# zhu-xlab/PFST

Hardware: AMD Instinct MI355X
Metric: PFST train-step images/s on 1024² IRRG tiles (higher is better)
Workload: dtype f32 (f16x3 split MFMA: two scaled fp16 pieces per operand, three products, fp32 accumulate); 1 GPU; pfst_pots_irrg2vaih_irrg_deeplabv3plus_r50-d8; global_batch=8, per_gpu_batch=8, tile=1024x1024x3, num_classes=6, parallelism=dp1, weights=seeded random init, conv_math=f16x3

## Files before the change

pfst_amd/csrc/conv_f16x3.hip:

```cpp
#include "conv_epilogue.h"
#include "amax.h"
#include "det.h"
#include "weight_jobs.h"
#include <math.h>
#include <stdlib.h>
#include <type_traits>
#include <utility>
#include "../../include/pfst_hip.h"

typedef _Float16 f16x8 __attribute__((ext_vector_type(8)));
typedef float f32x4 __attribute__((ext_vector_type(4)));

namespace {

constexpr int BN = 128;
constexpr int NP = 2;

template <int... Is, class F>
__device__ __forceinline__ void static_for_seq(std::integer_sequence<int, Is...>, F&& f) {
  (f(std::integral_constant<int, Is>()), ...);
}
template <int N, class F>
__device__ __forceinline__ void static_for(F&& f) {
  static_for_seq(std::make_integer_sequence<int, N>(), static_cast<F&&>(f));
// ... 73 lines not shown
  else if constexpr (op == 4)
    asm volatile("v_fma_mixlo_f16 %0, %1, %2, -%3 op_sel:[0,0,0] op_sel_hi:[0,0,1]" : "=v"(st.l[q]) : "v"(v[2 * q]), "s"(s), "v"(st.h[q]));
  else if constexpr (op == 5)
    asm volatile("v_fma_mixhi_f16 %0, %1, %2, -%3 op_sel:[0,0,1] op_sel_hi:[0,0,1]" : "+v"(st.l[q]) : "v"(v[2 * q + 1]), "s"(s), "v"(st.h[q]));
}
#endif

template <int K>
__device__ __forceinline__ void unpack_op_f16(const float (&v)[8], SplitF16& st) {
  constexpr int q = K & 3;
  if constexpr (K < 4) asm volatile("v_perm_b32 %0, %1, %2, %3" : "=v"(st.h[q]) : "v"(v[2 * q + 1]), "v"(v[2 * q]), "s"(0x05040100u));
  else asm volatile("v_perm_b32 %0, %1, %2, %3" : "=v"(st.l[q]) : "v"(v[2 * q + 1]), "v"(v[2 * q]), "s"(0x07060302u));
}

__global__ void pack_weight_f16x2_kernel(const float* __restrict__ w, uint4* __restrict__ wf, uint4* __restrict__ wd, int Cout, int Cin, int T,
                                         i64 set_in, i64 set_out, const float* __restrict__ amax) {
  w += blockIdx.y * set_in;
  if (wf) wf += blockIdx.y * set_out;
  if (wd) wd += blockIdx.y * set_out;
  const float s = scale_of(amax_exponent(amax_read(amax + (i64)blockIdx.y * PFST_AMAX_SUB)));
  const i64 nf = (i64)(T * Cin / 16) * 2 * Cout, nd = (i64)(T * Cout / 16) * 2 * Cin;
  for (i64 i = (i64)blockIdx.x * blockDim.x + threadIdx.x; i < nf + nd; i += (i64)gridDim.x * blockDim.x) {
    const bool dg = i >= nf;
    const i64 e = dg ? i - nf : i;
    const int M = dg ? Cin : Cout, Cq = dg ? Cout : Cin;
    if ((dg ? wd : wf) == nullptr) continue;
    if (Cq % 16 != 0) continue;
    const int row = (int)(e % M);
    const i64 gh = e / M;
    const int h = (int)(gh & 1);
    const int g = (int)(gh >> 1);
    float v[8];
#pragma unroll
    for (int j = 0; j < 8; ++j) {
      const int k = g * 16 + h * 8 + j;
      const int t = k / Cq, c = k - t * Cq;
      const int co = dg ? c : row, ci = dg ? row : c;
      v[j] = w[((i64)co * Cin + ci) * T + t];
    }
    uint4 ph, pl;
    split8_f16(v, s, ph, pl);
    uint4* dst = dg ? wd : wf;
    const i64 base = (i64)g * 2 * NP * M;
    dst[base + (i64)(0 * 2 + h) * M + row] = ph;
    dst[base + (i64)(1 * 2 + h) * M + row] = pl;
  }
}

__global__ __launch_bounds__(256) void pack_weight_f16x2_batched_kernel(const pfst_weight_job_t* __restrict__ jobs, int njobs) {
  const pfst_weight_job_t J = jobs[weight_job_of_block(jobs, njobs, blockIdx.x)];
  const int lb = blockIdx.x - J.first_block;
  const int Cout = J.Cout, Cin = J.Cin, T = J.T;
  const i64 nf = J.dst_f ? (i64)(T * Cin / 16) * 2 * Cout : 0, nd = J.dst_d ? (i64)(T * Cout / 16) * 2 * Cin : 0;
  const int bps = (int)((nf + nd + 255) / 256);
  const int set = lb / bps;
  const i64 n = (i64)Cout * Cin * T;
  const float s = scale_of(amax_exponent(amax_read(J.amax_f + (i64)set * PFST_AMAX_SUB)));
  const i64 i = (i64)(lb - set * bps) * 256 + threadIdx.x;
  if (i >= nf + nd) return;
  const float* w = J.src + set * n;
  const bool dg = i >= nf;
  const i64 e = dg ? i - nf : i;
  const int M = dg ? Cin : Cout, Cq = dg ? Cout : Cin;
  const int row = (int)(e % M);
  const i64 gh = e / M;
  const int h = (int)(gh & 1);
  const int g = (int)(gh >> 1);
  float v[8];
#pragma unroll
  for (int j = 0; j < 8; ++j) {
    const int k = g * 16 + h * 8 + j;
    const int t = k / Cq, c = k - t * Cq;
    const int co = dg ? c : row, ci = dg ? row : c;
    v[j] = w[((i64)co * Cin + ci) * T + t];
  }
  uint4 ph, pl;
  split8_f16(v, s, ph, pl);
  uint4* dst = reinterpret_cast<uint4*>(dg ? J.dst_d : J.dst_f) + set * (4 * n / 16);
  const i64 base = (i64)g * 2 * NP * M;
  dst[base + (i64)(0 * 2 + h) * M + row] = ph;
  dst[base + (i64)(1 * 2 + h) * M + row] = pl;
}

struct PfstResGate {
  const float* g = nullptr;
  i64 g_bs = 0;
  const unsigned long long* mask = nullptr;
};

template <int SHAPE, int BNB = 0, bool BPACK = false, bool ONE = false, int BMT = 128, bool BNL = false>
__device__ __forceinline__ void conv_igemm_f16x3_body(
    const float* __restrict__ in, i64 in_bs, const uint4* __restrict__ wk4, const float* __restrict__ bias,
    float* __restrict__ out, i64 out_bs, int C, int Hi, int Wi, int M, int Ho, int Wo, int ks,
    int ca, int cb, int cc, int cdivv, int accumulate, float* __restrict__ stats, int stats_T,
    const float* __restrict__ w_amax, const float* __restrict__ in_amax, int Y, int Z, int chain, const PfstBnbArgs& bnb,
    const PfstResGate& gate, const float4* __restrict__ bnl = nullptr) {
  static_assert(!BNL || (BMT == 256 && ONE && !BPACK && BNB == 0), "normalise-on-load exists for the 256-row 1x1 forward tile");
  static_assert(SHAPE == 32, "one MFMA shape: v_mfma_f32_32x32x16_f16 (the 16x16x32 form of round 3 was removed in round 5)");
  static_assert(BMT == 128 || (BMT == 256 && SHAPE == 32 && ONE) || (BMT == 64 && SHAPE == 32 && BNB == 0 && !BPACK),
                "the 256-row tile exists for the pixel-to-pixel 32x32 loop, the 64-row tile for the plain 32x32 loop");
  constexpr int BM = BMT, WAVES_N = 2, NT = BM == 64 ? 256 : 2 * BM;
  constexpr int TMW = BM == 64 ? 1 : 2;
  constexpr int TPT = BM == 256 ? 1 : 2;
  constexpr int NA = 2 * (2 * NP * BM) / NT;
  constexpr int TILE_A = 2 * NP * BM, TILE_B = 2 * NP * BN;
  constexpr int PAIR_CHUNKS = 2 * TILE_A + 2 * TILE_B;
  constexpr int SMEM_CHUNKS = 2 * PAIR_CHUNKS;
  __shared__ uint4 smem[SMEM_CHUNKS];
  uint4* const As = smem;
  uint4* const Bs = smem + 2 * TILE_A;

  const int tid = threadIdx.x, lane = tid & 63, wid = __builtin_amdgcn_readfirstlane(tid >> 6);
  const int wm0 = (wid / WAVES_N) * (32 * TMW), wn0 = (wid % WAVES_N) * 64;
  const int P = Ho * Wo, HiWi = Hi * Wi;
  constexpr int BNL_ROWS = 2048 + 32;
  __shared__ uint4 bnl_s[BNL ? BNL_ROWS / 2 : 1];
  if constexpr (BNL) {
    for (int i = tid; i < BNL_ROWS; i += NT) {
      const float4 cf = i < C ? bnl[i] : make_float4(0.f, 0.f, 0.f, 0.f);
      reinterpret_cast<float2*>(bnl_s)[i] = make_float2(cf.z, cf.w);
    }
    __syncthreads();
  }
  const int gx = (P + BN - 1) / BN, gy = (M + BM - 1) / BM, X = gx * gy;
  const int total = X * Y * Z, G = gridDim.x;
  auto decode = [&](int lin, int& bx, int& by, int& y, int& n) {
    const int zy = lin / X, x = lin - zy * X;
    y = zy / Z;
    const int z = zy - y * Z;
    n = y * Z + z;
    pfst_tile_order(x, gx, gy, !ONE && ks == 3, bx, by);
  };
  const int spt = (C + 31) / 32;
  const int ntaps = ONE ? 1 : ks * ks;
  const int KP = spt * ntaps;
  const int KT16 = (C / 16) * ntaps;
  const bool CHAIN = ONE && SHAPE == 32 && (KP & 1) == 0 && (chain & 1) != 0;
  float* const stats_mm = (stats && (chain & 2)) ? stats + (i64)2 * M * stats_T : nullptr;
#ifdef PFST_NT_ALL_K
  const bool nt_out = (chain & 4) != 0;
#else
  const bool nt_out = KP <= 16 && (chain & 4) != 0;
#endif

  const int pix = tid & (BN - 1), kh = (tid >> 7) & 1;
  const int bt = BM == 256 ? tid >> 8 : 0;
  const int a_seg = tid / BM, a_row = tid - a_seg * BM;
  constexpr unsigned OOB = 0x80000000u;
  const int a_chunk = 2 * M * 16, a_tile = 2 * NP * M * 16, b_chan = HiWi * 4;
  const int chan_step = 32 * HiWi * 4;

  int ld_lin = blockIdx.x;
  __amdgpu_buffer_rsrc_t a_rsrc, b_rsrc;
  unsigned a_voff;
  int ld_oy, ld_ox;
  bool ld_pvalid;
  auto set_load_side = [&](int lin) {
    int bx, by, y, n;
    decode(lin, bx, by, y, n);
    const int p = bx * BN + pix, m0 = by * BM;
    ld_pvalid = p < P;
    if constexpr (ONE) {
      ld_oy = p;
      ld_ox = 0;
    } else {
      ld_oy = ld_pvalid ? p / Wo : 0;
      ld_ox = ld_pvalid ? p - ld_oy * Wo : 0;
    }
    a_voff = (m0 + a_row < M) ? 16u * ((unsigned)a_seg * (unsigned)M + (unsigned)(m0 + a_row)) : OOB;
    a_rsrc = __builtin_amdgcn_make_buffer_rsrc(const_cast<uint4*>(wk4) + (i64)y * KT16 * 2 * NP * M, 0, KT16 * 2 * NP * M * 16, 0x00020000);
    b_rsrc = __builtin_amdgcn_make_buffer_rsrc(const_cast<float*>(in) + (i64)n * in_bs, 0, C * HiWi * 4, 0x00020000);
  };
  auto tap_voff = [&](int tap) -> unsigned {
    if constexpr (ONE) return ld_pvalid ? 4u * ((unsigned)(bt * 16 + kh * 8) * (unsigned)HiWi + (unsigned)ld_oy) : OOB;
    const int ty = tap / ks, tx = tap - ty * ks;
    int sy, sx;
    const bool ok = ld_pvalid & src_coord(ld_oy, ty, ca, cb, cc, cdivv, Hi, sy) & src_coord(ld_ox, tx, ca, cb, cc, cdivv, Wi, sx);
    return ok ? 4u * ((unsigned)(kh * 8) * (unsigned)HiWi + (unsigned)(sy * Wi + sx)) : OOB;
  };

  uint4 areg[2][NA];
  float breg[2][TPT][8];
  pfst_f32x16 acc32[TMW][2];
#pragma unroll
  for (int i = 0; i < TMW; ++i)
#pragma unroll
    for (int j = 0; j < 2; ++j)
#pragma unroll
      for (int r = 0; r < 16; ++r) acc32[i][j][r] = 0.f;

  auto load_b = [&](auto vc, auto setc, unsigned voff, int soff) {
    constexpr int v = decltype(vc)::value, SET = decltype(setc)::value;
    breg[SET][v >> 3][v & 7] = __builtin_bit_cast(float, __builtin_amdgcn_raw_buffer_load_b32(b_rsrc, voff, soff + ((v >> 3) * 16 + (v & 7)) * b_chan, 0));
  };
  auto load_a = [&](auto vc, auto setc, int a_soff) {
    constexpr int v = decltype(vc)::value, SET = decltype(setc)::value;
    areg[SET][v] = __builtin_bit_cast(uint4, __builtin_amdgcn_raw_buffer_load_b128(a_rsrc, a_voff, a_soff + (v / (NA / 2)) * a_tile + (v % (NA / 2)) * a_chunk, 0));
// ... 83 lines not shown
    uint4 cfr[BNL ? 4 : 1];
    const int cf_at = BNL ? sidx1 * 16 + bt * 8 + kh * 4 : 0;
    auto filler = [&](auto sc) {
      constexpr int m = decltype(sc)::value;
      if constexpr (m < 8) {
        if constexpr (TPT == 2) {
          load_b(std::integral_constant<int, 2 * m>(), std::integral_constant<int, SETL>(), voff2, soff2);
          load_b(std::integral_constant<int, 2 * m + 1>(), std::integral_constant<int, SETL>(), voff2, soff2);
        } else {
          load_b(std::integral_constant<int, m>(), std::integral_constant<int, SETL>(), voff2, soff2);
        }
      }
      if constexpr (m >= 8 && m < 8 + NA) As[NXT + ((m - 8) / (NA / 2)) * TILE_A + tid + NT * ((m - 8) % (NA / 2))] = areg[SETN][m - 8];
      if constexpr (BNL && m >= 8 && m < 12) cfr[m - 8] = bnl_s[cf_at + (m - 8)];
      if constexpr (m >= 12) {
        constexpr int SPS = 2 * TPT;
        static_for<SPS>([&](auto kc) {
          constexpr int kk = (m - 12) * SPS + decltype(kc)::value;
          if constexpr (BPACK) {
            if constexpr (kk < 8) unpack_op_f16<kk>(breg[SETN][0], s0);
            else if constexpr (kk < 16 && TPT == 2) unpack_op_f16<kk - 8>(breg[SETN][TPT - 1], s1);
          } else {
            if constexpr (BNL && kk < 24 && kk % 6 < 2) {
              constexpr int e = 2 * (kk / 6) + kk % 6;
              const uint4 c2 = cfr[e >> 1];
              const float sc = __builtin_bit_cast(float, (e & 1) ? c2.z : c2.x), sh = __builtin_bit_cast(float, (e & 1) ? c2.w : c2.y);
              breg[SETN][0][e] = fmaxf(__fmaf_rn(breg[SETN][0][e], sc, sh), 0.f);
            }
            if constexpr (kk < 24) split_op_f16<kk>(breg[SETN][0], sb, s0);
            else split_op_f16<kk - 24>(breg[SETN][TPT - 1], sb, s1);
          }
        });
      }
      if constexpr (m >= 12 && m < 12 + NA) load_a(std::integral_constant<int, m - 12>(), std::integral_constant<int, SETL>(), a_soff2);
      if constexpr (m == 18 && TPT == 2) {
        Bs[NXT + (0 * 2 + kh) * BN + pix] = make_uint4(s0.h[0], s0.h[1], s0.h[2], s0.h[3]);
        Bs[NXT + (1 * 2 + kh) * BN + pix] = make_uint4(s0.l[0], s0.l[1], s0.l[2], s0.l[3]);
      }
      if constexpr (m == 23 && TPT == 2) {
        Bs[NXT + TILE_B + (0 * 2 + kh) * BN + pix] = make_uint4(s1.h[0], s1.h[1], s1.h[2], s1.h[3]);
        Bs[NXT + TILE_B + (1 * 2 + kh) * BN + pix] = make_uint4(s1.l[0], s1.l[1], s1.l[2], s1.l[3]);
      }
      if constexpr (m == 23 && TPT == 1) {
        Bs[NXT + bt * TILE_B + (0 * 2 + kh) * BN + pix] = make_uint4(s0.h[0], s0.h[1], s0.h[2], s0.h[3]);
        Bs[NXT + bt * TILE_B + (1 * 2 + kh) * BN + pix] = make_uint4(s0.l[0], s0.l[1], s0.l[2], s0.l[3]);
      }
    };
    static_for<12 * TMW>([&](auto mc) {
      constexpr int m = decltype(mc)::value;
      constexpr int prod = m / (4 * TMW), rem = m % (4 * TMW), t = rem / (2 * TMW), i = (rem >> 1) % TMW, j = rem & 1;
      constexpr int pa = prod == 0 ? 1 : 0, pb = prod == 1 ? 1 : 0;
      acc32[i][j] = __builtin_amdgcn_mfma_f32_32x32x16_f16(af[t][i][pa], bf[t][j][pb], acc32[i][j], 0, 0, 0);
      if constexpr (PRE + m < 4 * RG) read_frag(std::integral_constant<int, PRE + m>());
      if constexpr (TMW == 2) {
        filler(std::integral_constant<int, m>());
      } else {
        filler(std::integral_constant<int, 2 * m>());
        filler(std::integral_constant<int, 2 * m + 1>());
      }
      __builtin_amdgcn_sched_barrier(0);
    });
    advance();
    __syncthreads();
  };
  auto epilogue = [&](int lin) {
    int bx, by, y, n;
    decode(lin, bx, by, y, n);
    if (y != ea_y) {
      ea = amax_exponent(amax_read(w_amax + (i64)y * PFST_AMAX_SUB));
      ea_y = y;
    }
    const int p0 = bx * BN, m0 = by * BM;
    float* const outn = out + (i64)n * out_bs;
    const float* const gsrc = gate.g ? gate.g + (i64)n * gate.g_bs : nullptr;
    const unsigned long long* const gmask = gate.g ? gate.mask + (i64)n * M * (P >> 6) : nullptr;
    const float ua = unscale_of(ea), ub = unscale_of(eb);
    {
#pragma unroll
      for (int i = 0; i < TMW; ++i)
#pragma unroll
        for (int j = 0; j < 2; ++j)
#pragma unroll
          for (int r = 0; r < 16; ++r) acc32[i][j][r] = acc32[i][j][r] * ua * ub;
      if constexpr (BNB != 0) {
        static_assert(PAIR_CHUNKS * sizeof(uint4) >= (NT / 64) * PFST_ROWSUM_LDS_FLOATS * sizeof(float), "epilogue scratch must fit into one pair buffer");
        conv_epilogue<2, 2, WAVES_N, BN, BNB, true>(acc32, outn, bias, stats, stats_T, accumulate, M, P, m0, p0, wm0, wn0, bx, n, wid, lane, bnb,
                                                    reinterpret_cast<float*>(smem + PAIR_CHUNKS), gsrc, gmask, nullptr, nt_out);
        __syncthreads();
      } else {
#ifdef PFST_STATS_LDSRED
        if (stats && !stats_mm && BMT != 64) {
          conv_epilogue<TMW, 2, WAVES_N, BN, 0, true>(acc32, outn, bias, stats, stats_T, accumulate, M, P, m0, p0, wm0, wn0, bx, n, wid, lane, PfstBnbArgs(),
                                                      reinterpret_cast<float*>(smem + PAIR_CHUNKS), gsrc, gmask, nullptr, nt_out);
          __syncthreads();
        } else
#endif
        conv_epilogue<TMW, 2, WAVES_N, BN>(acc32, outn, bias, stats, stats_T, accumulate, M, P, m0, p0, wm0, wn0, bx, n, wid, lane, PfstBnbArgs(), nullptr,
                                           gsrc, gmask, stats_mm, nt_out);
      }
#pragma unroll
      for (int i = 0; i < TMW; ++i)
#pragma unroll
        for (int j = 0; j < 2; ++j)
#pragma unroll
          for (int r = 0; r < 16; ++r) acc32[i][j][r] = 0.f;
    }
  };

  for (int lin = blockIdx.x; lin < total; lin += G) {
    if (!CHAIN || lin == (int)blockIdx.x) prologue(lin);
    for (int k = 0; k < KP; k += 2) {
      step32(std::integral_constant<int, 1>(), k);
      if (k + 1 < KP) step32(std::integral_constant<int, 0>(), k + 1);
    }
    epilogue(lin);
  }
}

template <int SHAPE, bool BPACK = false, bool ONE = false, int BMT = 128>
__global__ __launch_bounds__(BMT == 64 ? 256 : 2 * BMT, BMT == 256 ? 1 : 2) void conv_igemm_f16x3_kernel(
    const float* __restrict__ in, i64 in_bs, const uint4* __restrict__ wk4, const float* __restrict__ bias,
    float* __restrict__ out, i64 out_bs, int C, int Hi, int Wi, int M, int Ho, int Wo, int ks,
    int ca, int cb, int cc, int cdivv, int accumulate, float* __restrict__ stats, int stats_T,
    const float* __restrict__ w_amax, const float* __restrict__ in_amax, int Y, int Z, int chain, PfstResGate gate) {
  conv_igemm_f16x3_body<SHAPE, 0, BPACK, ONE, BMT>(in, in_bs, wk4, bias, out, out_bs, C, Hi, Wi, M, Ho, Wo, ks, ca, cb, cc, cdivv, accumulate, stats, stats_T,
                               w_amax, in_amax, Y, Z, chain, PfstBnbArgs(), gate);
}
__global__ __launch_bounds__(512, 1) void conv_igemm_f16x3_bnl_kernel(
    const float* __restrict__ in, i64 in_bs, const uint4* __restrict__ wk4, const float* __restrict__ bias,
    float* __restrict__ out, i64 out_bs, int C, int Hi, int Wi, int M, int Ho, int Wo, int ks,
    int ca, int cb, int cc, int cdivv, int accumulate, float* __restrict__ stats, int stats_T,
    const float* __restrict__ w_amax, const float* __restrict__ in_amax, int Y, int Z, int chain, const float4* __restrict__ bnl) {
  conv_igemm_f16x3_body<32, 0, false, true, 256, true>(in, in_bs, wk4, bias, out, out_bs, C, Hi, Wi, M, Ho, Wo, ks, ca, cb, cc, cdivv, accumulate, stats,
                                                       stats_T, w_amax, in_amax, Y, Z, chain, PfstBnbArgs(), PfstResGate(), bnl);
}
template <int BNB, bool ONE = false, int BMT = 128>
__global__ __launch_bounds__(2 * BMT, BMT == 128 ? 2 : 1) void conv_igemm_f16x3_bnb_kernel(
    const float* __restrict__ in, i64 in_bs, const uint4* __restrict__ wk4, const float* __restrict__ bias,
    float* __restrict__ out, i64 out_bs, int C, int Hi, int Wi, int M, int Ho, int Wo, int ks,
    int ca, int cb, int cc, int cdivv, int accumulate, float* __restrict__ stats, int stats_T,
    const float* __restrict__ w_amax, const float* __restrict__ in_amax, int Y, int Z, int chain, PfstBnbArgs bnb, PfstResGate gate) {
  conv_igemm_f16x3_body<32, BNB, false, ONE, BMT>(in, in_bs, wk4, bias, out, out_bs, C, Hi, Wi, M, Ho, Wo, ks, ca, cb, cc, cdivv, accumulate, stats, stats_T,
                                 w_amax, in_amax, Y, Z, chain, bnb, gate);
}


typedef float f32x16 __attribute__((ext_vector_type(16)));

struct Split4 {
  unsigned h[2], l[2];
  float t0[2], t1[2];
};
#ifdef PFST_F16X3_SPLIT6
template <int K>
__device__ __forceinline__ void split4_op_f16(const float (&v)[4], float s, Split4& st) {
  constexpr int q = K / 6, op = K % 6;
  if constexpr (op == 0) asm volatile("v_mul_f32 %0, %1, %2" : "=v"(st.t0[q]) : "s"(s), "v"(v[2 * q]));
  else if constexpr (op == 1) asm volatile("v_mul_f32 %0, %1, %2" : "=v"(st.t1[q]) : "s"(s), "v"(v[2 * q + 1]));
  else if constexpr (op == 2) asm volatile("v_cvt_pk_f16_f32 %0, %1, %2" : "=v"(st.h[q]) : "v"(st.t0[q]), "v"(st.t1[q]));
  else if constexpr (op == 3)
    asm volatile("v_fma_mix_f32 %0, %1, %2, -%3 op_sel:[0,0,0] op_sel_hi:[0,0,1]" : "=v"(st.t0[q]) : "v"(v[2 * q]), "s"(s), "v"(st.h[q]));
  else if constexpr (op == 4)
    asm volatile("v_fma_mix_f32 %0, %1, %2, -%3 op_sel:[0,0,1] op_sel_hi:[0,0,1]" : "=v"(st.t1[q]) : "v"(v[2 * q + 1]), "s"(s), "v"(st.h[q]));
  else asm volatile("v_cvt_pk_f16_f32 %0, %1, %2" : "=v"(st.l[q]) : "v"(st.t0[q]), "v"(st.t1[q]));
}
#else
template <int K>
__device__ __forceinline__ void split4_op_f16(const float (&v)[4], float s, Split4& st) {
  constexpr int q = K / 6, op = K % 6;
  if constexpr (op == 2) asm volatile("v_fma_mixlo_f16 %0, %1, %2, 0 op_sel_hi:[0,0,0]" : "=v"(st.h[q]) : "v"(v[2 * q]), "s"(s));
  else if constexpr (op == 3) asm volatile("v_fma_mixhi_f16 %0, %1, %2, 0 op_sel_hi:[0,0,0]" : "+v"(st.h[q]) : "v"(v[2 * q + 1]), "s"(s));
  else if constexpr (op == 4)
    asm volatile("v_fma_mixlo_f16 %0, %1, %2, -%3 op_sel:[0,0,0] op_sel_hi:[0,0,1]" : "=v"(st.l[q]) : "v"(v[2 * q]), "s"(s), "v"(st.h[q]));
  else if constexpr (op == 5)
    asm volatile("v_fma_mixhi_f16 %0, %1, %2, -%3 op_sel:[0,0,1] op_sel_hi:[0,0,1]" : "+v"(st.l[q]) : "v"(v[2 * q + 1]), "s"(s), "v"(st.h[q]));
}
#endif
template <int K>
__device__ __forceinline__ void unpack4_op_f16(const float (&v)[4], Split4& st) {
  constexpr int q = K & 1;
  if constexpr (K < 2) asm volatile("v_perm_b32 %0, %1, %2, %3" : "=v"(st.h[q]) : "v"(v[2 * q + 1]), "v"(v[2 * q]), "s"(0x05040100u));
  else asm volatile("v_perm_b32 %0, %1, %2, %3" : "=v"(st.l[q]) : "v"(v[2 * q + 1]), "v"(v[2 * q]), "s"(0x07060302u));
}

template <bool PACK, int BMT = 128, bool BNL = false>
__global__ __launch_bounds__(2 * BMT, BMT == 128 ? 2 : 1) void conv_wgrad_f16x3_line_kernel(
    const float* __restrict__ x, i64 x_bs, const float* __restrict__ dy, i64 dy_bs, float* __restrict__ dw,
    int J, int M, int P, int chunks, int chunk_len, int N, i64 x_gs, i64 dy_gs, i64 dw_gs, int gx, int gy, int gz,
    const float* __restrict__ x_amax, const float* __restrict__ dy_amax, const float4* __restrict__ bnl) {
  static_assert(!BNL || !PACK, "a pre-split operand is already normalised");
  constexpr int BM = BMT, BJ = 128, WM = 64, WAVES_N = 2, WN = 64, TM = 2, TN = 2, NT = 2 * BM;
  constexpr int RPP = NT / 8;
  constexpr int PA = BM / RPP, PB = BJ / RPP;
  constexpr int ROWS_A = BM + 2, ROWS_B = BJ + 2;
  constexpr int TILE_A = 4 * ROWS_A + 4, TILE_B = 4 * ROWS_B + 4;
  __shared__ uint4 As[2][2 * TILE_A];
  __shared__ uint4 Bs[2][2 * TILE_B];

  const int tid = threadIdx.x, lane = tid & 63, wid = __builtin_amdgcn_readfirstlane(tid >> 6);
  const int wm0 = (wid / WAVES_N) * WM, wn0 = (wid % WAVES_N) * WN;
  int bx, by, bz;
  {
    const int lin = blockIdx.x, tiles = gx * gy, z8 = gz & ~7;
    if (lin < tiles * z8) {
      const int xcd = lin & 7, idx = lin >> 3;
      const int sl = idx / tiles, t = idx - sl * tiles;
      bz = sl * 8 + xcd;
      by = t / gx;
      bx = t - by * gx;
    } else {
      bz = lin / tiles;
      const int t = lin - bz * tiles;
      by = t / gx;
      bx = t - by * gx;
    }
  }
  const int j0 = bx * BJ, m0 = by * BM;
// ... 220 lines not shown
  PFST_CHECK_LAUNCH();
  return PFST_OK;
}

extern "C" int pfst_absmax(const float* x, long long n, int planes, long long plane_stride, int slot_stride, float* slots,
                           pfst_stream_t stream) {
  PFST_CHECK_ARG(x && slots && n > 0 && planes > 0 && planes <= 65535 && (slot_stride == 0 || slot_stride == 1));
  int gx = (int)((n / 4 + 255) / 256);
  if (gx < 1) gx = 1;
  const int cap = planes > 1 ? 256 : 2048;
  if (gx > cap) gx = cap;
  hipLaunchKernelGGL(absmax_kernel, dim3(gx, planes), dim3(256), 0, (hipStream_t)stream, x, (i64)n, (i64)plane_stride, slot_stride, slots);
  PFST_CHECK_LAUNCH();
  return PFST_OK;
}

extern "C" int pfst_conv_pack_weight_f16x2(const float* w, void* wk4_fprop, void* wk4_dgrad, int Cout, int Cin, int T, int sets,
                                           const float* amax, pfst_stream_t stream) {
  PFST_CHECK_ARG(w && amax && (wk4_fprop || wk4_dgrad) && Cout > 0 && Cin > 0 && (T == 1 || T == 9) && sets >= 1 && sets <= 65535);
  PFST_CHECK_ARG(!wk4_fprop || Cin % 16 == 0);
  PFST_CHECK_ARG(!wk4_dgrad || Cout % 16 == 0);
  PFST_CHECK_ARG(sets == 1 || T == 1);
  const i64 n = (i64)Cout * Cin * T;
  int gx = ew_grid(n / 8 + 1);
  if (gx > 4096) gx = 4096;
  hipLaunchKernelGGL(pack_weight_f16x2_kernel, dim3(gx, sets), dim3(256), 0, (hipStream_t)stream, w, (uint4*)wk4_fprop, (uint4*)wk4_dgrad,
                     Cout, Cin, T, n, 4 * n / 16, amax);
  PFST_CHECK_LAUNCH();
  return PFST_OK;
}

extern "C" int pfst_conv_pack_weight_f16x2_batched(const pfst_weight_job_t* jobs_host, const pfst_weight_job_t* jobs_dev, int njobs,
                                                   pfst_stream_t stream) {
  PFST_CHECK_ARG(jobs_host && jobs_dev && njobs > 0);
  i64 blocks = 0;
  for (int j = 0; j < njobs; ++j) {
    const pfst_weight_job_t& J = jobs_host[j];
    PFST_CHECK_ARG(J.src && J.amax_f && (J.dst_f || J.dst_d) && J.Cout > 0 && J.Cin > 0 && (J.T == 1 || J.T == 9) && J.sets >= 1);
    PFST_CHECK_ARG((!J.dst_f || J.Cin % 16 == 0) && (!J.dst_d || J.Cout % 16 == 0) && (J.sets == 1 || J.T == 1) && J.first_block == blocks);
    blocks += weight_job_blocks(J, 1);
  }
  PFST_CHECK_ARG(blocks < (1ll << 31));
  hipLaunchKernelGGL(pack_weight_f16x2_batched_kernel, dim3((unsigned)blocks), dim3(256), 0, (hipStream_t)stream, jobs_dev, njobs);
  PFST_CHECK_LAUNCH();
  return PFST_OK;
}

extern "C" int pfst_conv_igemm_f16x3(const float* in, long long in_bs, const void* wk4, const float* w_amax, const float* in_amax,
                                     const float* bias, float* out, long long out_bs, int N, int C, int Hi, int Wi, int M, int Ho, int Wo,
                                     int ksize, int stride, int dil, int pad, int mode, int accumulate, float* stats,
                                     const pfst_bnb_fuse_t* bnb, const float* gate_dy, long long gate_dy_bs,
                                     const unsigned long long* gate_mask, int stats_minmax, const float* bnl, pfst_stream_t stream) {
  PFST_CHECK_ARG(in && wk4 && w_amax && in_amax && out && N > 0 && C > 0 && M > 0 && Hi > 0 && Wi > 0 && Ho > 0 && Wo > 0);
  PFST_CHECK_ARG(!bnl || (mode == 0 && ksize == 1 && stride == 1 && pad == 0 && M % 256 == 0 && C <= 2048 && !bias && !gate_dy && !(bnb && bnb->x) &&
                          !accumulate));
  PFST_CHECK_ARG(!stats_minmax || (stats && !bias && !(bnb && bnb->x)));
  PfstResGate gate;
  if (gate_dy) {
    PFST_CHECK_ARG(gate_mask && mode == 1 && !accumulate && !bias && !stats && M % 128 == 0 && ((i64)Ho * Wo) % 256 == 0 &&
                   gate_dy_bs >= (i64)M * Ho * Wo);
    gate.g = gate_dy;
    gate.g_bs = gate_dy_bs;
    gate.mask = gate_mask;
  }
  PFST_CHECK_ARG(!bnb || (bnb->x && bnb->x_bs >= (i64)M * Ho * Wo && (!bnb->y || bnb->y_bs >= (i64)M * Ho * Wo)));
  PFST_CHECK_ARG(!bnb || !bnb->y_mask || (bnb->y && bnb->relu && ((i64)Ho * Wo) % 256 == 0));
  PFST_CHECK_ARG((ksize == 1 || ksize == 3) && (stride == 1 || stride == 2) && dil >= 1 && pad >= 0 && (mode == 0 || mode == 1));
  PFST_CHECK_ARG(in_bs >= (i64)C * Hi * Wi && out_bs >= (i64)M * Ho * Wo && N <= 65535);
  PFST_CHECK_ARG((i64)C * Hi * Wi * 4 < (1ll << 31) && (i64)M * Ho * Wo * 4 < (1ll << 31) && (i64)ksize * ksize * C * M * 4 < (1ll << 31));
  if ((C % 32 != 0 && !(ksize == 1 && C % 16 == 0)) || M <= 32) {
    pfst_set_error(__FILE__, __LINE__, "f16x3 kernel needs C % 32 == 0 (1x1: C % 16 == 0) and more than 32 output channels (use pfst_conv_igemm_split)");
    return PFST_ERR_UNSUPPORTED;
  }
  const bool small = M <= 64;
  PFST_CHECK_ARG(!small || !(bnb && bnb->x));
  const int span = (ksize - 1) * dil;
  if (mode == 0) {
    PFST_CHECK_ARG(Ho == (Hi + 2 * pad - span - 1) / stride + 1 && Wo == (Wi + 2 * pad - span - 1) / stride + 1);
  } else {
    PFST_CHECK_ARG(Hi == (Ho + 2 * pad - span - 1) / stride + 1 && Wi == (Wo + 2 * pad - span - 1) / stride + 1);
  }
  int a, b, c, d;
  if (mode == 0) { a = stride; b = dil; c = -pad; d = 1; } else { a = 1; b = -dil; c = pad; d = stride; }
  const int stats_T = N * (int)cdiv((i64)Ho * Wo, BN) * 2;
  const bool one = !small && ksize == 1 && stride == 1 && pad == 0;
  const bool big = one && M % 256 == 0;
  const i64 total = (i64)cdiv((i64)Ho * Wo, BN) * cdiv(M, big ? 256 : small ? 64 : 128) * N;
  PFST_CHECK_ARG(total < (1ll << 31));
  const dim3 grid(f16x3_grid(total, one && ((C + 31) / 32) % 2 == 0, big ? 1 : 2));
  const int chain = 1 | (stats_minmax ? 2 : 0) | 4;
  if (bnb && bnb->x) {
    PFST_CHECK_ARG(M % 128 == 0 && !bias && !stats && bnb->coef && bnb->partials);
#define PFST_LAUNCH_F16_BNB(MODE_, ONE_)                                                                                                    \
    hipLaunchKernelGGL((conv_igemm_f16x3_bnb_kernel<MODE_, ONE_>), grid, dim3(256), 0, (hipStream_t)stream, in, (i64)in_bs, (const uint4*)wk4, bias, \
                       out, (i64)out_bs, C, Hi, Wi, M, Ho, Wo, ksize, a, b, c, d, accumulate, stats, stats_T, w_amax, in_amax, 1, N, chain, *bnb, gate)
#define PFST_LAUNCH_F16_BNB_BIG(MODE_)                                                                                                      \
    hipLaunchKernelGGL((conv_igemm_f16x3_bnb_kernel<MODE_, true, 256>), grid, dim3(512), 0, (hipStream_t)stream, in, (i64)in_bs, (const uint4*)wk4, bias, \
                       out, (i64)out_bs, C, Hi, Wi, M, Ho, Wo, ksize, a, b, c, d, accumulate, stats, stats_T, w_amax, in_amax, 1, N, chain, *bnb, gate)
    if (big) {
      if (!bnb->relu) PFST_LAUNCH_F16_BNB_BIG(3);
      else if (bnb->y_mask) PFST_LAUNCH_F16_BNB_BIG(4);
      else if (bnb->y) PFST_LAUNCH_F16_BNB_BIG(2);
      else PFST_LAUNCH_F16_BNB_BIG(1);
    } else if (one) {
      if (!bnb->relu) PFST_LAUNCH_F16_BNB(3, true);
      else if (bnb->y_mask) PFST_LAUNCH_F16_BNB(4, true);
      else if (bnb->y) PFST_LAUNCH_F16_BNB(2, true);
      else PFST_LAUNCH_F16_BNB(1, true);
    } else {
      if (!bnb->relu) PFST_LAUNCH_F16_BNB(3, false);
      else if (bnb->y_mask) PFST_LAUNCH_F16_BNB(4, false);
      else if (bnb->y) PFST_LAUNCH_F16_BNB(2, false);
      else PFST_LAUNCH_F16_BNB(1, false);
    }
#undef PFST_LAUNCH_F16_BNB
#undef PFST_LAUNCH_F16_BNB_BIG
    PFST_CHECK_LAUNCH();
    return PFST_OK;
  }
  if (bnl)
    hipLaunchKernelGGL(conv_igemm_f16x3_bnl_kernel, grid, dim3(512), 0, (hipStream_t)stream, in, (i64)in_bs, (const uint4*)wk4, bias, out, (i64)out_bs, C, Hi, Wi,
                       M, Ho, Wo, ksize, a, b, c, d, accumulate, stats, stats_T, w_amax, in_amax, 1, N, chain, reinterpret_cast<const float4*>(bnl));
  else if (small)
    hipLaunchKernelGGL((conv_igemm_f16x3_kernel<32, false, false, 64>), grid, dim3(256), 0, (hipStream_t)stream, in, (i64)in_bs, (const uint4*)wk4, bias, out,
                       (i64)out_bs, C, Hi, Wi, M, Ho, Wo, ksize, a, b, c, d, accumulate, stats, stats_T, w_amax, in_amax, 1, N, chain, gate);
  else if (big)
    hipLaunchKernelGGL((conv_igemm_f16x3_kernel<32, false, true, 256>), grid, dim3(512), 0, (hipStream_t)stream, in, (i64)in_bs, (const uint4*)wk4, bias, out,
                       (i64)out_bs, C, Hi, Wi, M, Ho, Wo, ksize, a, b, c, d, accumulate, stats, stats_T, w_amax, in_amax, 1, N, chain, gate);
  else if (one)
    hipLaunchKernelGGL((conv_igemm_f16x3_kernel<32, false, true>), grid, dim3(256), 0, (hipStream_t)stream, in, (i64)in_bs, (const uint4*)wk4, bias, out,
                       (i64)out_bs, C, Hi, Wi, M, Ho, Wo, ksize, a, b, c, d, accumulate, stats, stats_T, w_amax, in_amax, 1, N, chain, gate);
  else
    hipLaunchKernelGGL(conv_igemm_f16x3_kernel<32>, grid, dim3(256), 0, (hipStream_t)stream, in, (i64)in_bs, (const uint4*)wk4, bias, out,
                       (i64)out_bs, C, Hi, Wi, M, Ho, Wo, ksize, a, b, c, d, accumulate, stats, stats_T, w_amax, in_amax, 1, N, chain, gate);
  PFST_CHECK_LAUNCH();
  return PFST_OK;
}

extern "C" int pfst_wino_gemm_f16x3(const float* V, const void* U4, const float* u_amax, const float* v_amax, float* Mbuf, int N, int K,
                                    int M, int T, int m, int v_packed, pfst_stream_t stream) {
  PFST_CHECK_ARG(V && U4 && u_amax && v_amax && Mbuf && N > 0 && N <= 65535 && K > 0 && K % 32 == 0 && M > 64 && T > 0 && (m == 2 || m == 4));
  const int nx = (m + 2) * (m + 2);
  PFST_CHECK_ARG((i64)K * T * 4 < (1ll << 31) && (i64)M * T * 4 < (1ll << 31) && (i64)K * M * 4 < (1ll << 31));
  const bool big = M % 256 == 0;
  const i64 total = (i64)cdiv((i64)T, BN) * cdiv(M, big ? 256 : 128) * nx * N;
  PFST_CHECK_ARG(total < (1ll << 31));
  const dim3 grid(f16x3_grid(total, (K / 32) % 2 == 0, big ? 1 : 2));
  const int chain = 1 | 4;
  if (big && v_packed)
    hipLaunchKernelGGL((conv_igemm_f16x3_kernel<32, true, true, 256>), grid, dim3(512), 0, (hipStream_t)stream, V, (i64)K * T, (const uint4*)U4,
                       (const float*)nullptr, Mbuf, (i64)M * T, K, 1, T, M, 1, T, 1, 1, 1, 0, 1, 0, (float*)nullptr, 0, u_amax, v_amax, nx, N, chain, PfstResGate());
  else if (big)
    hipLaunchKernelGGL((conv_igemm_f16x3_kernel<32, false, true, 256>), grid, dim3(512), 0, (hipStream_t)stream, V, (i64)K * T, (const uint4*)U4,
                       (const float*)nullptr, Mbuf, (i64)M * T, K, 1, T, M, 1, T, 1, 1, 1, 0, 1, 0, (float*)nullptr, 0, u_amax, v_amax, nx, N, chain, PfstResGate());
  else if (v_packed)
    hipLaunchKernelGGL((conv_igemm_f16x3_kernel<32, true, true>), grid, dim3(256), 0, (hipStream_t)stream, V, (i64)K * T, (const uint4*)U4,
                       (const float*)nullptr, Mbuf, (i64)M * T, K, 1, T, M, 1, T, 1, 1, 1, 0, 1, 0, (float*)nullptr, 0, u_amax, v_amax, nx, N, chain, PfstResGate());
  else
    hipLaunchKernelGGL((conv_igemm_f16x3_kernel<32, false, true>), grid, dim3(256), 0, (hipStream_t)stream, V, (i64)K * T, (const uint4*)U4, (const float*)nullptr,
                       Mbuf, (i64)M * T, K, 1, T, M, 1, T, 1, 1, 1, 0, 1, 0, (float*)nullptr, 0, u_amax, v_amax, nx, N, chain, PfstResGate());
  PFST_CHECK_LAUNCH();
  return PFST_OK;
}

int pfst_wgrad_f16x3_launch(const float* x, i64 x_bs, const float* dy, i64 dy_bs, float* dw, int N, int J, int M, int P, int groups,
                            i64 x_gs, i64 dy_gs, i64 dw_gs, const float* x_amax, const float* dy_amax, int packed, hipStream_t s, const float* bnl) {
// ... 51 lines not shown
```

Baseline: 29.99 images/s.

## Compute strided 1x1 transposed conv as a dense GEMM with scatter epilogue

For the data-gradient of a stride-2 1x1 convolution (mode 1), it runs a dense pixel-to-pixel GEMM over the small input grid only. A new epilogue scatters each result to the even output positions and writes zeros to the neighbouring odd positions with 64-bit buffer stores. This avoids iterating over the three quarters of output pixels that receive no contribution and the implicit-GEMM address logic for them. In exchange it adds a specialised kernel variant, and in accumulate mode it leaves the untouched positions as they were.

```diff
diff --git a/pfst_amd/csrc/conv_f16x3.hip b/pfst_amd/csrc/conv_f16x3.hip
--- a/pfst_amd/csrc/conv_f16x3.hip
+++ b/pfst_amd/csrc/conv_f16x3.hip
@@ -179,13 +179,61 @@
   dst[base + (i64)(1 * 2 + h) * M + row] = pl;
 }
 
+template <int TM>
+__device__ __forceinline__ void scatter2_epilogue(pfst_f32x16 (&acc)[TM][2], float* __restrict__ out, int accumulate, int M, int Pin, int Wi,
+                                                  int m0, int p0, int wm0, int wn0, int lane) {
+  typedef unsigned u32x2 __attribute__((ext_vector_type(2)));
+  constexpr unsigned OOB = 0x80000000u;
+  const int l31 = lane & 31, lh = lane >> 5;
+  const int Pout = 4 * Pin, Wo = 2 * Wi;
+  const __amdgpu_buffer_rsrc_t rsrc = __builtin_amdgcn_make_buffer_rsrc(out, 0, M * Pout * 4, 0x00020000);
+  unsigned voff[2], voff_below[2];
+#pragma unroll
+  for (int j = 0; j < 2; ++j) {
+    const int pp = p0 + wn0 + j * 32 + l31;
+    const int iy = pp / Wi, ix = pp - iy * Wi;
+    const unsigned at = 4u * ((unsigned)(2 * Wo * iy + 2 * ix) + 4u * (unsigned)lh * (unsigned)Pout);
+    voff[j] = pp < Pin ? at : OOB;
+    voff_below[j] = pp < Pin ? at + 4u * (unsigned)Wo : OOB;
+  }
+  const int row0 = m0 + wm0;
+#pragma unroll
+  for (int i = 0; i < TM; ++i)
+#pragma unroll
+    for (int j = 0; j < 2; ++j) {
+      if (accumulate) {
+        float old[16];
+#pragma unroll
+        for (int r = 0; r < 16; ++r)
+          old[r] = __builtin_bit_cast(float, __builtin_amdgcn_raw_buffer_load_b32(rsrc, voff[j], 4 * Pout * (row0 + i * 32 + (r & 3) + 8 * (r >> 2)), 0));
+#pragma unroll
+        for (int r = 0; r < 16; ++r) {
+          const float v = acc[i][j][r] + old[r];
+          __builtin_amdgcn_raw_buffer_store_b32(__builtin_bit_cast(unsigned, v), rsrc, voff[j], 4 * Pout * (row0 + i * 32 + (r & 3) + 8 * (r >> 2)), 0);
+        }
+      } else {
+#pragma unroll
+        for (int r = 0; r < 16; ++r) {
+          const float v = acc[i][j][r];
+          const int soff = 4 * Pout * (row0 + i * 32 + (r & 3) + 8 * (r >> 2));
+          u32x2 top, zero;
+          top.x = __builtin_bit_cast(unsigned, v);
+          top.y = 0u;
+          zero.x = zero.y = 0u;
+          __builtin_amdgcn_raw_buffer_store_b64(top, rsrc, voff[j], soff, 0);
+          __builtin_amdgcn_raw_buffer_store_b64(zero, rsrc, voff_below[j], soff, 0);
+        }
+      }
+    }
+}
+
 struct PfstResGate {
   const float* g = nullptr;
   i64 g_bs = 0;
   const unsigned long long* mask = nullptr;
 };
 
-template <int SHAPE, int BNB = 0, bool BPACK = false, bool ONE = false, int BMT = 128, bool BNL = false>
+template <int SHAPE, int BNB = 0, bool BPACK = false, bool ONE = false, int BMT = 128, bool BNL = false, bool SCAT = false>
 __device__ __forceinline__ void conv_igemm_f16x3_body(
     const float* __restrict__ in, i64 in_bs, const uint4* __restrict__ wk4, const float* __restrict__ bias,
     float* __restrict__ out, i64 out_bs, int C, int Hi, int Wi, int M, int Ho, int Wo, int ks,
@@ -193,6 +241,7 @@
     const float* __restrict__ w_amax, const float* __restrict__ in_amax, int Y, int Z, int chain, const PfstBnbArgs& bnb,
     const PfstResGate& gate, const float4* __restrict__ bnl = nullptr) {
   static_assert(!BNL || (BMT == 256 && ONE && !BPACK && BNB == 0), "normalise-on-load exists for the 256-row 1x1 forward tile");
+  static_assert(!SCAT || (ONE && !BPACK && BNB == 0 && !BNL && BMT != 64), "the scattering epilogue exists for the plain pixel-to-pixel tiles");
   static_assert(SHAPE == 32, "one MFMA shape: v_mfma_f32_32x32x16_f16 (the 16x16x32 form of round 3 was removed in round 5)");
   static_assert(BMT == 128 || (BMT == 256 && SHAPE == 32 && ONE) || (BMT == 64 && SHAPE == 32 && BNB == 0 && !BPACK),
                 "the 256-row tile exists for the pixel-to-pixel 32x32 loop, the 64-row tile for the plain 32x32 loop");
@@ -209,7 +258,7 @@
 
   const int tid = threadIdx.x, lane = tid & 63, wid = __builtin_amdgcn_readfirstlane(tid >> 6);
   const int wm0 = (wid / WAVES_N) * (32 * TMW), wn0 = (wid % WAVES_N) * 64;
-  const int P = Ho * Wo, HiWi = Hi * Wi;
+  const int HiWi = Hi * Wi, P = SCAT ? HiWi : Ho * Wo;
   constexpr int BNL_ROWS = 2048 + 32;
   __shared__ uint4 bnl_s[BNL ? BNL_ROWS / 2 : 1];
   if constexpr (BNL) {
@@ -459,7 +508,9 @@
         for (int j = 0; j < 2; ++j)
 #pragma unroll
           for (int r = 0; r < 16; ++r) acc32[i][j][r] = acc32[i][j][r] * ua * ub;
-      if constexpr (BNB != 0) {
+      if constexpr (SCAT) {
+        scatter2_epilogue<TMW>(acc32, outn, accumulate, M, P, Wi, m0, p0, wm0, wn0, lane);
+      } else if constexpr (BNB != 0) {
         static_assert(PAIR_CHUNKS * sizeof(uint4) >= (NT / 64) * PFST_ROWSUM_LDS_FLOATS * sizeof(float), "epilogue scratch must fit into one pair buffer");
         conv_epilogue<2, 2, WAVES_N, BN, BNB, true>(acc32, outn, bias, stats, stats_T, accumulate, M, P, m0, p0, wm0, wn0, bx, n, wid, lane, bnb,
                                                     reinterpret_cast<float*>(smem + PAIR_CHUNKS), gsrc, gmask, nullptr, nt_out);
@@ -510,6 +561,13 @@
     const float* __restrict__ w_amax, const float* __restrict__ in_amax, int Y, int Z, int chain, const float4* __restrict__ bnl) {
   conv_igemm_f16x3_body<32, 0, false, true, 256, true>(in, in_bs, wk4, bias, out, out_bs, C, Hi, Wi, M, Ho, Wo, ks, ca, cb, cc, cdivv, accumulate, stats,
                                                        stats_T, w_amax, in_amax, Y, Z, chain, PfstBnbArgs(), PfstResGate(), bnl);
+}
+template <int BMT>
+__global__ __launch_bounds__(2 * BMT, BMT == 128 ? 2 : 1) void conv_igemm_f16x3_scat_kernel(
+    const float* __restrict__ in, i64 in_bs, const uint4* __restrict__ wk4, float* __restrict__ out, i64 out_bs, int C, int Hi, int Wi, int M,
+    int accumulate, const float* __restrict__ w_amax, const float* __restrict__ in_amax, int Z, int chain) {
+  conv_igemm_f16x3_body<32, 0, false, true, BMT, false, true>(in, in_bs, wk4, nullptr, out, out_bs, C, Hi, Wi, M, 2 * Hi, 2 * Wi, 1, 1, 1, 0, 1, accumulate,
+                                                              nullptr, 0, w_amax, in_amax, 1, Z, chain, PfstBnbArgs(), PfstResGate());
 }
 template <int BNB, bool ONE = false, int BMT = 128>
 __global__ __launch_bounds__(2 * BMT, BMT == 128 ? 2 : 1) void conv_igemm_f16x3_bnb_kernel(
@@ -896,6 +954,21 @@
   }
   int a, b, c, d;
   if (mode == 0) { a = stride; b = dil; c = -pad; d = 1; } else { a = 1; b = -dil; c = pad; d = stride; }
+  if (mode == 1 && !small && ksize == 1 && stride == 2 && pad == 0 && Ho == 2 * Hi && Wo == 2 * Wi && M % 128 == 0 && !bias && !stats &&
+      !(bnb && bnb->x) && !gate_dy && (((uintptr_t)out | (uintptr_t)((i64)out_bs * 4)) & 7) == 0) {
+    const bool big_s = M % 256 == 0;
+    const i64 tiles = (i64)cdiv((i64)Hi * Wi, BN) * (M / (big_s ? 256 : 128)) * N;
+    PFST_CHECK_ARG(tiles < (1ll << 31));
+    const dim3 grid_s(f16x3_grid(tiles, ((C + 31) / 32) % 2 == 0, big_s ? 1 : 2));
+    if (big_s)
+      hipLaunchKernelGGL((conv_igemm_f16x3_scat_kernel<256>), grid_s, dim3(512), 0, (hipStream_t)stream, in, (i64)in_bs, (const uint4*)wk4, out, (i64)out_bs,
+                         C, Hi, Wi, M, accumulate, w_amax, in_amax, N, 1);
+    else
+      hipLaunchKernelGGL((conv_igemm_f16x3_scat_kernel<128>), grid_s, dim3(256), 0, (hipStream_t)stream, in, (i64)in_bs, (const uint4*)wk4, out, (i64)out_bs,
+                         C, Hi, Wi, M, accumulate, w_amax, in_amax, N, 1);
+    PFST_CHECK_LAUNCH();
+    return PFST_OK;
+  }
   const int stats_T = N * (int)cdiv((i64)Ho * Wo, BN) * 2;
   const bool one = !small && ksize == 1 && stride == 1 && pad == 0;
   const bool big = one && M % 256 == 0;
```

Result: no change. 30.11 images/s (median of 6 runs) (+0.4%).
